# DaehwanKimLab/tophat

Measured on AMD Instinct MI355X. Metric: paired reads/sec through segment_juncs+long_spanning_reads; junctions.bed diff=0, higher is better.
Workload: dtype u64

## Files before the change

### tophat_amd/csrc/thj_ctx.h

```cpp
#pragma once
#include <hip/hip_runtime.h>
#include <cstdint>
#include <utility>
#include <vector>

#include "../../include/thj.h"
#include "thj_core.h"
#include "thj_internal.h"
#include "thj_jbknown_core.h"

using thj::u64;

#define HIPCHK(expr)                                                                          \
    do {                                                                                      \
        hipError_t e__ = (expr);                                                              \
        if (e__ != hipSuccess) {                                                              \
            thj_set_error("%s: %s (%s:%d)", #expr, hipGetErrorString(e__), __FILE__, __LINE__); \
            return THJ_EHIP;                                                                  \
        }                                                                                     \
    } while (0)

struct OwnedSpanBatch {
    thj_span_batch desc;
    void* ptrs[8];
    size_t reads_infl_bytes;
};

template <class T> struct DevBuf { T* p = nullptr; int64_t cap = 0; void release() { (void)hipFree(p); p = nullptr; cap = 0; } };
struct JbStore { DevBuf<u64> w64; DevBuf<uint32_t> w32; DevBuf<unsigned long long> cnt; int64_t cap = 0; void release() { w64.release(); w32.release(); cnt.release(); cap = 0; } };
struct JbOcc; struct JbiOcc; struct JbfOcc; struct JbfUOcc; struct JbfJOcc; struct JbbRec;
struct JbState {
    int64_t want = 0, records = 0;
    jbk::ReadFilter flt{};
    struct Junc { JbStore tab; DevBuf<u64> sorted; DevBuf<JbOcc> occ; int64_t occ_used = 0; DevBuf<u64> known; int64_t n_known = 0; std::vector<thj_juncstat> rows; } junc;
    struct Indel { bool on = false; JbStore tab; DevBuf<JbiOcc> occ; int64_t occ_used = 0; std::vector<thj_insstat> ins; std::vector<thj_juncstat> del; } indel;
    struct Fus { bool on = false; int32_t anchor = 20, mismatches = 2, multireads = 2; JbStore tab; DevBuf<uint32_t> grp; int64_t groups = 0;
                 DevBuf<JbfOcc> focc; DevBuf<JbfUOcc> uocc; DevBuf<JbfJOcc> jocc; std::vector<thj_fusstat> rows; } fus;
    struct Best { bool on = false; int32_t max_multihits = 20, suppress = 0, max_penalty = 6; DevBuf<JbbRec> rec; DevBuf<u64> skey; DevBuf<uint8_t> keep;
                  DevBuf<unsigned long long> cnt; int64_t counts[4] = {0, 0, 0, 0}; } best;
};

struct CovState {
    int64_t n_blocks = 0; int32_t n_contigs = 0;
    DevBuf<u64> bits; DevBuf<int32_t> extent;
    unsigned long long* d_found = nullptr;
    DevBuf<uint32_t> rec_len; DevBuf<u64> rec_seq; int64_t n_reads = 0;
    uint32_t* d_ext_off = nullptr; DevBuf<u64> ext_val; DevBuf<u64> filter; u64 filter_mask = 0;
    struct List {
        u64 *key = nullptr, *key2 = nullptr; uint32_t *skip = nullptr, *skip2 = nullptr; int64_t cap = 0;
        void release() { (void)hipFree(key); (void)hipFree(key2); (void)hipFree(skip); (void)hipFree(skip2); *this = List(); }
    } list;
    DevBuf<thj_mx_cand> mx_cand; int64_t n_mx_cand = 0;
    int32_t min_intron = 0, max_intron = 0; bool pending = false;
    void release() {
        bits.release(); extent.release(); rec_len.release(); rec_seq.release(); ext_val.release(); filter.release(); list.release(); mx_cand.release();
        (void)hipFree(d_found); (void)hipFree(d_ext_off); *this = CovState();
    }
};

struct thj_ctx {
    int device = 0;
    hipStream_t stream = nullptr;
    bool own_stream = false;
    hipStream_t aux_stream[2] = {};
    double aux_ratio[2] = {0, 0}; bool aux_independent[2] = {false, false};
    const u64* d_blocks = nullptr; bool own_blocks = false;
    uint32_t* d_contig_blk = nullptr; int32_t* d_contig_len = nullptr;
    std::vector<uint32_t> h_contig_blk; std::vector<int64_t> h_lens;
    int32_t n_contigs = 0; int64_t n_blocks = 0;
    int64_t junc_cap = 0, indel_cap = 0;
    u64 *d_junc = nullptr, *d_del = nullptr, *d_ins_key = nullptr, *d_ins_val = nullptr;
    unsigned int* d_ovf = nullptr;
    unsigned long long* d_cnt = nullptr;
    u64 *d_junc_sorted = nullptr, *d_del_sorted = nullptr, *d_ins_key_sorted = nullptr, *d_ins_val_sorted = nullptr;
    u64 *d_tmp_keys = nullptr, *d_tmp_vals = nullptr, *d_tmp_keys2 = nullptr;
    int64_t out_cap_junc = 0, out_cap_indel = 0;
    unsigned long long* d_out_n = nullptr;
    unsigned long long* h_pinned = nullptr;
    void* d_sort_tmp = nullptr; size_t sort_tmp_bytes = 0;
    int64_t n_junc = 0, n_del = 0, n_ins = 0;
    hipEvent_t probe_ev = nullptr; bool probe_pending = false;
    uint8_t* d_fus_ignore = nullptr; int64_t n_fus_ignore = 0;
    struct SjSet {
        uint32_t* d_rescue_list = nullptr; int64_t rescue_list_cap = 0;
        uint32_t* d_many = nullptr;
        void* d_lists = nullptr; size_t lists_cap = 0;
        int32_t* d_rescue_slots = nullptr;
        hipEvent_t ev_flat = nullptr, ev_side = nullptr;
    } sj_set[2];
    uint32_t* d_junc_bucket = nullptr; int64_t n_junc_buckets = 0;
    u64* d_span_cat = nullptr;
    u64* d_span_junc = nullptr; int64_t n_span_junc = 0; int64_t cap_span_junc = 0;
    u64* d_span_ins_key = nullptr; uint32_t* d_span_ins_seq = nullptr; int64_t n_span_ins = 0; int64_t cap_span_ins = 0;
    void* d_huge_ws = nullptr; uint32_t* d_huge_list = nullptr; int huge_blocks = 0, huge_list_cap = 0;
    void* d_span_fus = nullptr; int64_t n_span_fus = 0; int64_t cap_span_fus = 0;
    void* d_aln_pool = nullptr; void* d_aln_sorted = nullptr; int64_t aln_cap = 0;
    u64* d_aln_keys = nullptr;
    unsigned long long* d_aln_count = nullptr; unsigned int* d_span_status = nullptr;
    int64_t n_alns = 0, n_ovf = 0, span_reads = 0, ovf_cap = 0;
    uint8_t* d_nrec = nullptr;
    std::vector<thj_aln> h_alns;
    struct SpanSet { uint32_t* d_worklist = nullptr; int64_t worklist_cap = 0; void* d_ent = nullptr; int64_t ent_cap = 0; void* d_joined = nullptr; int64_t joined_cap = 0; uint32_t* d_defer = nullptr; int64_t defer_cap = 0; };
    SpanSet span_set[2]; int span_last_set = 0;
    bool span_t0_pending = false; int64_t span_t0_n[2] = {0, 0}; hipEvent_t span_t0_prof[2][32] = {};
    hipEvent_t span_ev[10] = {};
    bool span_profile = false;
    std::vector<std::pair<hipEvent_t, hipEvent_t>> span_prof_events;
    CovState cov;
    thj_fusion* d_fus = nullptr; unsigned long long* d_fus_count = nullptr; int64_t fus_cap = 0;
    hipEvent_t fus_probe_ev = nullptr; bool fus_probe_pending = false;
    std::vector<thj_fusion> h_fusions;
    thj_fusion* d_fus_out = nullptr; int64_t n_fus_out = 0;
    bool h_fus_stale = false;
    struct DevBlock { void* p; size_t cap; bool used; };
    std::vector<DevBlock> dev_cache; size_t dev_cache_bytes = 0;
    void* d_ing0 = nullptr; size_t ing_cap0 = 0; void* d_ing1 = nullptr; size_t ing_cap1 = 0;
    thj_juncdb_target* d_juncdb = nullptr; int64_t n_juncdb = 0;
    bool juncdb_has_fus = false, juncdb_fusion_on = false;
    uint8_t* d_bam = nullptr; size_t bam_cap = 0; int64_t bam_bytes = 0;
    void* d_bam_tmp = nullptr; size_t bam_tmp_cap = 0;
    uint8_t* d_contig_names = nullptr; uint32_t* d_contig_name_off = nullptr; uint32_t* d_contig_name_sorted = nullptr; int32_t n_contig_names = 0;
    void* d_infl_tmp = nullptr; size_t infl_tmp_cap = 0;
    JbState jb;
    struct thj_comm* xchg = nullptr;
    bool profile = false;
    bool serial_launch = false;
    std::vector<std::pair<hipEvent_t, hipEvent_t>> prof_events;
    std::vector<hipEvent_t> prof_all; std::vector<int> prof_sets;
    std::vector<hipEvent_t> event_pool;
};
template <class T, class C>
static inline int grow_device_buffer(T*& ptr, C& cap, C new_cap, size_t bytes) {
    if (ptr) HIPCHK(hipDeviceSynchronize());
    (void)hipFree(ptr); ptr = nullptr; cap = 0;
    HIPCHK(hipMalloc((void**)&ptr, bytes));
    cap = new_cap;
    return THJ_OK;
}
static inline int ensure_sort_tmp(struct thj_ctx* c, size_t need) {
    return need > c->sort_tmp_bytes ? grow_device_buffer(c->d_sort_tmp, c->sort_tmp_bytes, need, need) : THJ_OK;
}
template <class Run>
static inline int run_with_sort_tmp(struct thj_ctx* c, Run run) {
    size_t need = 0;
    HIPCHK(run(nullptr, need));
    if (const int e = ensure_sort_tmp(c, need)) return e;
    size_t bytes = c->sort_tmp_bytes;
    HIPCHK(run(c->d_sort_tmp, bytes));
    return THJ_OK;
}
template <class T>
static inline int read_device_value(struct thj_ctx* c, const T* d, T* h) {
    HIPCHK(hipMemcpyAsync(h, d, sizeof(T), hipMemcpyDeviceToHost, c->stream));
    HIPCHK(hipStreamSynchronize(c->stream));
    return THJ_OK;
}
struct DevTemps {
    std::vector<void**> slots;
    DevTemps() = default; DevTemps(const DevTemps&) = delete;
    template <class T> hipError_t alloc(T*& p, size_t bytes) { p = nullptr; slots.push_back((void**)&p); return hipMalloc((void**)&p, bytes); }
    ~DevTemps() { for (void** p : slots) { (void)hipFree(*p); *p = nullptr; } }
};
hipEvent_t thj_get_event(struct thj_ctx* c);
int thj_ensure_aux_streams(struct thj_ctx* c, int need);
void thj_warm_span(hipStream_t s); void thj_warm_ingest(hipStream_t s); void thj_warm_bamout(hipStream_t s);
int thj_dev_alloc(struct thj_ctx* c, void** out, size_t bytes);
void thj_dev_release(struct thj_ctx* c, void* p);
void thj_dev_cache_free(struct thj_ctx* c);
void thj_span_free(struct thj_ctx* c);
int thj_span_compact_device(struct thj_ctx* c, void** d_out);
void thj_bamout_free(struct thj_ctx* c);
struct thj_reported_recs { thj_aln* recs; int64_t n; const int64_t* ins_off; uint8_t* ins_bases; int64_t n_groups; uint32_t resume_member, resume_skip; };
// ... 5 lines not shown
```

### tophat_amd/csrc/thj_segjuncs.hip

```cpp
#include <hip/hip_runtime.h>
#include <hipcub/hipcub.hpp>

#include <cstdio>
#include <cstdlib>
#include <algorithm>
#include <cstring>
#include <cstddef>
#include <chrono>
#include <vector>

#include "../../include/thj.h"
#include "thj_core.h"
#include "thj_fusion_block.h"
#include "thj_internal.h"

using namespace thj;

static_assert(sizeof(thj_hit) == 16 && sizeof(Hit) == 16, "hit layout");
static_assert(sizeof(thj_params) == sizeof(Params), "params layout");




static constexpr u64 EMPTY = ~0ull;
// ... 1205 lines not shown
    if (!c->probe_pending || hipEventQuery(c->probe_ev) != hipSuccess) return THJ_OK;
    c->probe_pending = false;
    const unsigned long long* n = &c->h_pinned[32];
    const bool gj = n[CNT_JUNC] * 5 > (unsigned long long)c->junc_cap * 2;
    const bool gi = (n[CNT_DEL] > n[CNT_INS] ? n[CNT_DEL] : n[CNT_INS]) * 5 > (unsigned long long)c->indel_cap * 2;
    return (gj || gi) ? grow_tables(c, gj, gi) : THJ_OK;
}

extern "C" int thj_segjuncs_configure(thj_ctx* c, int64_t junc_capacity, int64_t indel_capacity) {
    if (!c || junc_capacity < 1 || indel_capacity < 1) { thj_set_error("thj_segjuncs_configure: bad argument"); return THJ_EINVAL; }
    HIPCHK(hipSetDevice(c->device));
    HIPCHK(hipStreamSynchronize(c->stream));
    int rc = alloc_tables(c, junc_capacity, indel_capacity);
    if (rc) return rc;
    return reset_tables_async(c);
}

extern "C" int thj_segjuncs_reset_async(thj_ctx* c) {
    if (!c) { thj_set_error("null ctx"); return THJ_EINVAL; }
    HIPCHK(hipSetDevice(c->device));
    return reset_tables_async(c);
}

static int check_params(const thj_params* p, const thj_seg_batch* b) {
    if (p->segment_length < 8 || p->segment_length > 64) {
        thj_set_error("segment_length %d unsupported by the device path (8..64: the 8 bases either side of a segment boundary "
                      "that make a support read must lie inside the segments, segment_juncs.cpp:3580-3584; a 2L read piece and an "
                      "L+16 support read must fit one 128-bit plane word)", p->segment_length);
        return THJ_EINVAL;
    }
    if (p->max_insertion_length > 6 || p->max_insertion_length < 0) { thj_set_error("max_insertion_length %d unsupported (0..6)", p->max_insertion_length); return THJ_EINVAL; }
    if (p->max_deletion_length < 0 || p->max_deletion_length > 1000000) { thj_set_error("max_deletion_length out of range"); return THJ_EINVAL; }
    if (p->max_segment_intron + p->segment_length + 64 >= (1 << 29)) { thj_set_error("max_segment_intron too large for the packed key"); return THJ_EINVAL; }
    if (b->nseg < 1 || b->nseg > 16) { thj_set_error("nseg %d unsupported (1..16)", b->nseg); return THJ_EINVAL; }
    if (b->words_per_plane < 1 || b->words_per_plane > 8) { thj_set_error("words_per_plane %d unsupported (1..8: reads of up to 512 bases)", b->words_per_plane); return THJ_EINVAL; }
    if (b->n_reads < 0 || (int64_t)b->n_reads + b->ordinal_base >= (1ll << 29)) { thj_set_error("batch too large: read ordinals must stay below 2^29"); return THJ_EINVAL; }
    return THJ_OK;
}

int thj_dev_alloc(thj_ctx* c, void** out, size_t bytes) {
    if (bytes < 256) bytes = 256;
    int best = -1;
    for (size_t i = 0; i < c->dev_cache.size(); ++i) {
        const thj_ctx::DevBlock& b = c->dev_cache[i];
        if (!b.used && b.cap >= bytes && b.cap <= 2 * bytes + 65536 && (best < 0 || b.cap < c->dev_cache[(size_t)best].cap)) best = (int)i;
    }
    if (best >= 0) { c->dev_cache[(size_t)best].used = true; *out = c->dev_cache[(size_t)best].p; return THJ_OK; }
    if (c->dev_cache_bytes > ((size_t)16 << 30)) {
        for (size_t i = 0; i < c->dev_cache.size();) {
            if (!c->dev_cache[i].used) { hipFree(c->dev_cache[i].p); c->dev_cache_bytes -= c->dev_cache[i].cap; c->dev_cache.erase(c->dev_cache.begin() + (ptrdiff_t)i); }
            else ++i;
        }
    }
    const size_t cap = bytes + bytes / 8;
    void* p = nullptr;
    HIPCHK(hipMalloc(&p, cap));
    c->dev_cache.push_back({p, cap, true});
    c->dev_cache_bytes += cap;
    *out = p;
    return THJ_OK;
}
void thj_dev_release(thj_ctx* c, void* p) {
    if (!p) return;
    for (auto& b : c->dev_cache) if (b.p == p) { b.used = false; return; }
    hipFree(p);
}
void thj_dev_cache_free(thj_ctx* c) {
    for (auto& b : c->dev_cache) hipFree(b.p);
    c->dev_cache.clear(); c->dev_cache_bytes = 0;
}

hipEvent_t thj_get_event(thj_ctx* c) {
    if (!c->event_pool.empty()) { hipEvent_t e = c->event_pool.back(); c->event_pool.pop_back(); return e; }
    hipEvent_t e;
    hipEventCreate(&e);
    return e;
}


struct SjGeom {
    int n_tiles, grid, seg_cap;
    int tmax; size_t xcap;
    int rgrid, mgrid; bool wide;
    int64_t slots() const { return (int64_t)grid * seg_cap; }
    int64_t rescue_slice_words() const { return slots(); }             int64_t rescue_shared_words() const { return 2 * (int64_t)MANY_CAP; }
    int64_t rescue_words() const { return rescue_slice_words() + rescue_shared_words() + MAX_LISTS; }
    size_t tq_bytes() const { return (size_t)slots() * tmax * 16; }    size_t xq_bytes() const { return xcap * 16; }
    size_t frl_bytes() const { return (size_t)slots() * 32; }
    size_t te_bytes() const { return (size_t)slots() * tmax * 4; }
    size_t gen_bytes() const { return (size_t)slots() * 4; }           size_t xe_bytes() const { return xcap * 4; }
    size_t cnt_bytes() const { return (size_t)grid * 12; }
    size_t lists_bytes() const { return tq_bytes() + xq_bytes() + frl_bytes() + te_bytes() + gen_bytes() + xe_bytes() + cnt_bytes() + 512; }
};
static SjGeom sj_geometry(const Params& p, const DevBatch& b) {
    SjGeom q{};
    q.n_tiles = (b.n_reads + TPB - 1) / TPB;
    q.grid = q.n_tiles < 256 * 8 - 1 ? q.n_tiles : 256 * 8 - 1;
    q.seg_cap = (q.n_tiles + q.grid - 1) / q.grid * TPB;
    q.tmax = (b.nseg > 2 ? b.nseg - 2 : 0) + (b.nseg - 1 > 2 * FLAT_MATES ? b.nseg - 1 : 2 * FLAT_MATES);
    q.xcap = (size_t)2 * (size_t)b.n_reads > ((size_t)1 << 20) ? (size_t)2 * (size_t)b.n_reads : ((size_t)1 << 20);
    if (getenv("THJ_XTASK_CAP")) q.xcap = (size_t)atoll(getenv("THJ_XTASK_CAP"));
    q.rgrid = q.grid < RESCUE_GRID ? q.grid : RESCUE_GRID; q.mgrid = q.n_tiles < MID_GRID ? q.n_tiles : MID_GRID; q.wide = p.segment_length > 32;
    return q;
}
static constexpr size_t SJ_MANY_BYTES = 32 + (size_t)MANY_CAP * 8;
static constexpr size_t SJ_SLOTS_BYTES = 16 + (size_t)HEAVY_CAP * 4;
static int ensure_sj_set(thj_ctx* c, int set, const SjGeom& q, bool mates) {
    thj_ctx::SjSet& ss = c->sj_set[set];
    const bool grow_rescue = ss.rescue_list_cap < q.rescue_words(), grow_lists = ss.lists_cap < q.lists_bytes();
    if ((grow_rescue || grow_lists) && getenv("THJ_TRACE"))
        fprintf(stderr, "[stage 1] scratch set %d grows:%s%s (%lld words, %zu bytes needed)\n", set, grow_rescue ? " rescue list" : "", grow_lists ? " list block" : "", (long long)q.rescue_words(), q.lists_bytes());
    if (grow_rescue) { const int rc = grow_device_buffer(ss.d_rescue_list, ss.rescue_list_cap, q.rescue_words(), (size_t)q.rescue_words() * 4); if (rc) return rc; }
    if (!ss.d_many) HIPCHK(hipMalloc((void**)&ss.d_many, SJ_MANY_BYTES));
    if (mates && !ss.d_rescue_slots) HIPCHK(hipMalloc((void**)&ss.d_rescue_slots, SJ_SLOTS_BYTES));
    if (grow_lists) { const size_t cap = q.lists_bytes() + q.lists_bytes() / 8; return grow_device_buffer(ss.d_lists, ss.lists_cap, cap, cap); }
    return THJ_OK;
}

struct SjPlan {
    int set; bool serial;
    hipStream_t s_main;
    hipStream_t s_side;
    hipEvent_t ev_flat;
    hipEvent_t ev_side;
    hipEvent_t m_flat[2];
};
static int sj_plan(thj_ctx* c, int set, SjPlan& pl) {
    static const bool serial_env = getenv("THJ_SJ_SERIAL") && atoi(getenv("THJ_SJ_SERIAL")) != 0;
    thj_ctx::SjSet& ss = c->sj_set[set];
    pl = SjPlan{}; pl.set = set; pl.serial = serial_env || c->serial_launch; pl.s_main = pl.s_side = c->stream;
    if (pl.serial) return THJ_OK;
    if (const int rc = thj_ensure_aux_streams(c, set + 1)) return rc;
    if (!ss.ev_flat) { HIPCHK(hipEventCreateWithFlags(&ss.ev_flat, hipEventDisableTiming)); HIPCHK(hipEventCreateWithFlags(&ss.ev_side, hipEventDisableTiming)); }
    pl.s_side = c->aux_stream[set]; pl.ev_flat = ss.ev_flat; pl.ev_side = ss.ev_side;
    return THJ_OK;
}

struct SjView { Genome g; Params p; DevBatch b; Tables t; RescueList rl; SjLists sl; XTasks x; SjGeom q; unsigned long long* cnt; };
static int sj_view(thj_ctx* c, const thj_params* tp, const thj_seg_batch* db, int set, SjView& v) {
    v.g = Genome{c->d_blocks, c->d_contig_blk, c->d_contig_len, c->n_contigs};
    memcpy(&v.p, tp, sizeof v.p); memcpy(&v.b, db, sizeof v.b);
    v.t = Tables{c->d_junc, (u64)c->junc_cap - 1, c->d_del, (u64)c->indel_cap - 1, c->d_ins_key, c->d_ins_val,
                 (u64)c->indel_cap - 1, junc_list(c), del_list(c), ins_list(c), c->d_ovf, c->d_cnt};
    v.cnt = c->d_cnt;
#ifdef THJ_EXP
    { int f = getenv("THJ_EXP_FLAGS") ? atoi(getenv("THJ_EXP_FLAGS")) : 0; HIPCHK(hipMemcpyToSymbol(HIP_SYMBOL(thj_exp_flags), &f, sizeof f)); }
#endif
    const SjGeom q = v.q = sj_geometry(v.p, v.b);
    if (const int rc = ensure_sj_set(c, set, q, v.b.mate_off != nullptr)) return rc;
    const thj_ctx::SjSet& ss = c->sj_set[set];
    unsigned int* const counts = (unsigned int*)ss.d_many;
    static const int many_min = getenv("THJ_MANY_HITS") ? atoi(getenv("THJ_MANY_HITS")) : MID_HITS;
    RescueList& rl = v.rl;
    rl.list = ss.d_rescue_list; rl.blk_cnt = ss.d_rescue_list + q.rescue_slice_words() + q.rescue_shared_words(); rl.seg_cap = q.seg_cap; rl.own_slice = q.grid;
    rl.many_min = many_min; rl.mid_min = many_min < GEN_HITS ? many_min : GEN_HITS;
    rl.many_count = counts; rl.many_list = ss.d_many + 8;
    rl.heavy_count = (unsigned int*)ss.d_rescue_slots; rl.heavy_list = ss.d_rescue_slots ? (uint32_t*)ss.d_rescue_slots + 4 : nullptr; rl.slot_pool = nullptr;
    SjLists& sl = v.sl; XTasks& x = v.x;
    char* at = (char*)ss.d_lists;
    auto take = [&at](size_t bytes) { char* const piece = at; at += bytes; return piece; };
    sl.tq = (uint4*)take(q.tq_bytes());            x.q = (uint4*)take(q.xq_bytes());
    sl.frl = (uint4*)take(q.frl_bytes());          sl.te = (uint32_t*)take(q.te_bytes());
    sl.gen = (uint32_t*)take(q.gen_bytes());       x.e = (uint32_t*)take(q.xe_bytes());
    sl.task_cnt = (unsigned int*)take(q.cnt_bytes()); sl.frl_cnt = sl.task_cnt + q.grid; sl.gen_cnt = sl.frl_cnt + q.grid;
    sl.task_cap = q.seg_cap * q.tmax;
    sl.mid_count = counts + 2; sl.mid_list = ss.d_many + 8 + MANY_CAP;
    x.count = counts + 3; x.cap = (unsigned int)(q.xcap < 0xFFFFFFFFull ? q.xcap : 0xFFFFFFFFull); x.ovf = c->d_ovf + 3;
    return THJ_OK;
}

static void launch_sj_flat(const SjView& v, hipStream_t s) {
    const dim3 grid((unsigned)v.q.grid), tpb(TPB);
    if (v.b.nseg <= 4) hipLaunchKernelGGL(thj_k_sj_flat<4>, grid, tpb, 0, s, v.p, v.b, v.rl, v.sl, v.cnt);
    else if (v.b.nseg <= 8) hipLaunchKernelGGL(thj_k_sj_flat<8>, grid, tpb, 0, s, v.p, v.b, v.rl, v.sl, v.cnt);
    else hipLaunchKernelGGL(thj_k_sj_flat<16>, grid, tpb, 0, s, v.p, v.b, v.rl, v.sl, v.cnt);
}
template <int HITS, int T, bool SLICED, int G>
static void launch_sj_general(const SjView& v, int grid, hipStream_t s) {
    if (v.b.nseg <= 8) hipLaunchKernelGGL((thj_k_sj_general<HITS, T, SLICED, 9, G>), dim3((unsigned)grid), dim3(T), 0, s, v.p, v.b, v.rl, v.sl, v.x, v.cnt);
    else hipLaunchKernelGGL((thj_k_sj_general<HITS, T, SLICED, 17, G>), dim3((unsigned)grid), dim3(T), 0, s, v.p, v.b, v.rl, v.sl, v.x, v.cnt);
}
static void launch_sj_tasks_list(const SjView& v, hipStream_t s) {
    if (v.q.wide) hipLaunchKernelGGL(thj_k_sj_tasks_list<true>, dim3(v.q.rgrid), dim3(TPB), 0, s, v.g, v.p, v.b, v.t, v.x);
    else hipLaunchKernelGGL(thj_k_sj_tasks_list<false>, dim3(v.q.rgrid), dim3(TPB), 0, s, v.g, v.p, v.b, v.t, v.x);
}
static void launch_sj_tasks(const SjView& v, hipStream_t s) {
    if (v.q.wide) hipLaunchKernelGGL(thj_k_sj_tasks<true>, dim3(v.q.grid), dim3(TPB), 0, s, v.g, v.p, v.b, v.t, v.sl);
    else hipLaunchKernelGGL(thj_k_sj_tasks<false>, dim3(v.q.grid), dim3(TPB), 0, s, v.g, v.p, v.b, v.t, v.sl);
}

static constexpr int SJ_PROF_N = 8;
static hipEvent_t sj_mark(thj_ctx* c, hipStream_t s) { if (!c->profile) return nullptr; hipEvent_t e = thj_get_event(c); hipEventRecord(e, s); c->prof_all.push_back(e); return e; }

static int sj_launch_flat(thj_ctx* c, SjPlan& pl, const SjView& v) {
    const thj_ctx::SjSet& ss = c->sj_set[pl.set];
    HIPCHK(hipMemsetAsync(ss.d_many, 0, 32, pl.s_main));
    HIPCHK(hipMemsetAsync(v.rl.blk_cnt + v.q.grid, 0, 4, pl.s_main));
    if (v.b.mate_off) HIPCHK(hipMemsetAsync(ss.d_rescue_slots, 0, 16, pl.s_main));
    pl.m_flat[0] = sj_mark(c, pl.s_main);
    launch_sj_flat(v, pl.s_main);
    pl.m_flat[1] = sj_mark(c, pl.s_main);
    if (!pl.serial) { HIPCHK(hipEventRecord(pl.ev_flat, pl.s_main)); HIPCHK(hipStreamWaitEvent(pl.s_side, pl.ev_flat, 0)); }
    HIPCHK(hipGetLastError());
    return THJ_OK;
}

static int sj_launch_rest(thj_ctx* c, const SjPlan& pl, const SjView& v) {
    const SjGeom& q = v.q;
    const hipStream_t sm = pl.s_main, sa = pl.s_side;
    hipEvent_t b0 = sj_mark(c, sa);
    hipLaunchKernelGGL(thj_k_segjuncs_shared, dim3(q.rgrid), dim3(TPB), 0, sa, v.p, v.b, v.rl, v.x, v.cnt);
    hipEvent_t b1 = sj_mark(c, sa);
    launch_sj_general<MID_HITS, MID_T, false, MID_G>(v, q.mgrid, sa);
    hipEvent_t c1 = sj_mark(c, sa);
    launch_sj_general<GEN_HITS, TPB, true, GEN_G>(v, q.grid, sa);
    hipEvent_t a1 = sj_mark(c, sa);
    if (v.b.mate_off) {
        hipLaunchKernelGGL(thj_k_segjuncs_rescue, dim3(q.rgrid), dim3(TPB), 0, sa, v.g, v.p, v.b, v.rl, q.grid + 1, v.x, v.cnt);
        hipLaunchKernelGGL(thj_k_segjuncs_rescue_shared, dim3(q.rgrid), dim3(TPB), 0, sa, v.g, v.p, v.b, v.rl, v.x, v.cnt);
    }
    hipEvent_t a4 = sj_mark(c, sa);
    launch_sj_tasks_list(v, sa);
    hipEvent_t a5 = sj_mark(c, sa);
    if (!pl.serial) HIPCHK(hipEventRecord(pl.ev_side, sa));
    hipEvent_t m2 = sj_mark(c, sm);
    if (v.b.mate_off) hipLaunchKernelGGL(thj_k_sj_rescue_flat, dim3(q.grid), dim3(TPB), 0, sm, v.g, v.p, v.b, v.sl, q.seg_cap, v.cnt, v.sl.mid_count + 2);
    hipEvent_t m3 = sj_mark(c, sm);
    launch_sj_tasks(v, sm);
    hipEvent_t m4 = sj_mark(c, sm);
    if (c->profile) {
        const std::pair<hipEvent_t, hipEvent_t> spans[SJ_PROF_N] = {{pl.m_flat[0], pl.m_flat[1]}, {c1, a1}, {b1, c1}, {b0, b1}, {a1, a4}, {a4, a5}, {m2, m3}, {m3, m4}};
        c->prof_events.insert(c->prof_events.end(), spans, spans + SJ_PROF_N);
        c->prof_sets.push_back(pl.set);
    }
    HIPCHK(hipGetLastError());
    return THJ_OK;
}

static int sj_join(const SjPlan& pl) { if (!pl.serial) HIPCHK(hipStreamWaitEvent(pl.s_main, pl.ev_side, 0)); return THJ_OK; }
static int sj_probe(thj_ctx* c) {
    if (!c->probe_ev) HIPCHK(hipEventCreateWithFlags(&c->probe_ev, hipEventDisableTiming));
    if (!c->probe_pending) {
        HIPCHK(hipMemcpyAsync(&c->h_pinned[32], c->d_cnt, CNT_N * sizeof(unsigned long long), hipMemcpyDeviceToHost, c->stream));
        HIPCHK(hipEventRecord(c->probe_ev, c->stream));
        c->probe_pending = true;
    }
    return THJ_OK;
}

extern "C" int thj_segjuncs_run_async(thj_ctx* c, const thj_params* tp, const thj_seg_batch* db) {
    if (!c || !tp || !db) { thj_set_error("thj_segjuncs_run_async: null argument"); return THJ_EINVAL; }
    if (!c->d_blocks) { thj_set_error("no genome resident: call thj_genome_upload/adopt first"); return THJ_ESTATE; }
    int rc = check_params(tp, db);
    if (rc) return rc;
    HIPCHK(hipSetDevice(c->device));
    if (db->n_reads == 0) return THJ_OK;
    if ((rc = maybe_grow_tables(c))) return rc;
    SjPlan pl; SjView v;
    if ((rc = sj_plan(c, 0, pl)) || (rc = sj_view(c, tp, db, 0, v)) || (rc = sj_launch_flat(c, pl, v)) || (rc = sj_launch_rest(c, pl, v)) || (rc = sj_join(pl))) return rc;
    return sj_probe(c);
}

extern "C" int thj_segjuncs_run_pair_async(thj_ctx* c, const thj_params* tp0, const thj_seg_batch* db0, const thj_params* tp1, const thj_seg_batch* db1) {
    if (!c || !tp0 || !db0 || !tp1 || !db1) { thj_set_error("thj_segjuncs_run_pair_async: null argument"); return THJ_EINVAL; }
    if (!c->d_blocks) { thj_set_error("no genome resident: call thj_genome_upload/adopt first"); return THJ_ESTATE; }
    int rc = check_params(tp0, db0);
    if (rc || (rc = check_params(tp1, db1))) return rc;
    HIPCHK(hipSetDevice(c->device));
    if ((rc = maybe_grow_tables(c))) return rc;
    const thj_params* const tp[2] = {tp0, tp1}; const thj_seg_batch* const db[2] = {db0, db1};
    SjPlan pl[2]; SjView v[2];
    for (int k = 0; k < 2; ++k) if (db[k]->n_reads && ((rc = sj_plan(c, k, pl[k])) || (rc = sj_view(c, tp[k], db[k], k, v[k])))) return rc;
    for (int k = 0; k < 2; ++k) if (db[k]->n_reads && (rc = sj_launch_flat(c, pl[k], v[k]))) return rc;
    if (db0->n_reads && (rc = sj_launch_rest(c, pl[0], v[0]))) return rc;
    if (db1->n_reads && (rc = sj_launch_rest(c, pl[1], v[1]))) { if (db0->n_reads) sj_join(pl[0]); return rc; }
    for (int k = 0; k < 2; ++k) if (db[k]->n_reads && (rc = sj_join(pl[k]))) return rc;
    return (db0->n_reads || db1->n_reads) ? sj_probe(c) : THJ_OK;
}

extern "C" int thj_profile_serial(thj_ctx* c, int on) {
    if (!c) { thj_set_error("null ctx"); return THJ_EINVAL; }
    HIPCHK(hipSetDevice(c->device));
    HIPCHK(hipStreamSynchronize(c->stream));
    c->serial_launch = on != 0;
    return THJ_OK;
}

extern "C" int thj_profile_segjuncs(thj_ctx* c, int enable, double* avg_ms, int64_t* launches, double* stats) {
    if (!c) { thj_set_error("null ctx"); return THJ_EINVAL; }
    HIPCHK(hipSetDevice(c->device));
    HIPCHK(hipStreamSynchronize(c->stream));
    double sum[SJ_PROF_N] = {0};
    const size_t n = c->prof_events.size() / SJ_PROF_N;
    for (size_t i = 0; i < c->prof_events.size(); ++i) {
// ... 465 lines not shown
```

### tophat_amd/csrc/thj_span.hip

```cpp
#include <hip/hip_runtime.h>
#include <hipcub/hipcub.hpp>

#include <cstdio>
#include <algorithm>
#include <cstdlib>
#include <cstring>
#include <cstddef>
#include <chrono>
#include <vector>

#include "../../include/thj.h"
#include "thj_span_core.h"
#include "thj_span_fusion.h"
#include "thj_ctx.h"
#include "thj_scan.h"

using namespace thj;


static_assert(sizeof(thj_span_hit) == 32 && sizeof(SpanHit) == 32, "span hit layout");
static_assert(sizeof(thj_aln) == 128 && sizeof(OutAln) == 128 && sizeof(thj_aln_slot) == 128 && offsetof(thj_aln_slot, cigar_hi) == 64, "aln layout");

struct DevSpanBatch {
    int32_t n_reads, nseg, W, qual_stride;
// ... 181 lines not shown
    for (int k = 0; k < IPT; ++k) { s_off[tid * IPT + k] = excl; excl += v[k]; }
    if (tid == 0) s_off[NS] = total;
    __syncthreads();
    return total;
}
__device__ __forceinline__ int slice_of(const unsigned int* s_off, int G, unsigned int i) {
    int lo = 0, hi = G;
    while (hi - lo > 1) { const int mid = (lo + hi) >> 1; if (s_off[mid] <= i) lo = mid; else hi = mid; }
    return lo;
}

template <int MS, int WPE = 4>
__global__ __launch_bounds__(256, WPE) void thj_k_stitch(Genome g, Params p, SpanSets S, DevSpanBatch b, RecSink sink, Tiers t, int G) {
    extern __shared__ uint4 lds_stage[];
    constexpr int NC = lean_classes(MS);
    __shared__ unsigned int s_off[NC * MAX_SLICES + 1];
    __shared__ unsigned int s_rec, s_fwd;
    if (threadIdx.x == 0) { s_rec = 0; s_fwd = 0; }
    unsigned int n_fwd = 0;
    SpanHitHead* stage = (SpanHitHead*)lds_stage + (size_t)threadIdx.x * b.nseg;
    const unsigned int total = slice_offsets<256, NC * MAX_SLICES>(t.blk_lean, NC * G, s_off);
    for (unsigned int i = blockIdx.x * 256 + threadIdx.x; i < total; i += gridDim.x * 256) {
        int sl = slice_of(s_off, NC * G, i);
        const int r = (int)t.wl_lean[(int64_t)sl * t.chunk + (i - s_off[sl])];
        int st = span_read_lean<MS>(g, p, S, b.hits, b.seg_off + (size_t)r * b.nseg, b.nseg, b.planes + (size_t)r * 3 * b.W, b.W,
                                (int)b.read_len[r], b.quals + (size_t)r * b.qual_stride, (uint32_t)r, stage, sink);
        if (st == SPAN_INCOMPAT) st = p.fusion_search ? SPAN_NEED_GENERIC : SPAN_OK;
        const bool fwd = st == SPAN_NEED_GENERIC;
        if (!fwd) { sink.done((uint32_t)r); if (st) atomicAdd(&sink.status[st], 1u); }
        sl %= G;
        for (unsigned long long todo = __ballot(fwd); todo;) {
            const int leader = __ffsll((long long)todo) - 1;
            const int sl_l = __shfl(sl, leader);
            const unsigned long long same = __ballot(fwd && sl == sl_l);
            const int lane = (int)(threadIdx.x & 63u);
            unsigned int base = 0;
            if (lane == leader) base = atomicAdd(&t.blk_multi[sl_l], (unsigned int)__popcll(same));
            base = (unsigned int)__shfl((int)base, leader);
            if (fwd && sl == sl_l) {
                t.wl_multi[(int64_t)sl * t.chunk + base + (unsigned int)__popcll(same & (lane ? (~0ull >> (64 - lane)) : 0ull))] = (uint32_t)r;
                ++n_fwd;
            }
            todo &= ~same;
        }
    }
    if (sink.acc) atomicAdd(&s_rec, (unsigned int)sink.acc);
    if (n_fwd) atomicAdd(&s_fwd, n_fwd);
    __syncthreads();
    if (threadIdx.x == 0 && s_rec) atomicAdd(sink.total, (unsigned long long)s_rec);
    if (threadIdx.x == 0 && s_fwd) atomicAdd(&t.counters[1], s_fwd);
}

struct LdsChainHits {
    const Q16* col;
    __device__ __forceinline__ SpanHit operator[](int s) const {
        const Q16 a = col[(2 * s) * 256], b = col[(2 * s + 1) * 256];
        SpanHit h;
        h.ref_id = a.x; h.left = (int32_t)a.y; h.meta = a.z; h.cigar[0] = a.w;
        h.cigar[1] = b.x; h.cigar[2] = b.y; h.cigar[3] = b.z; h.cigar[4] = b.w;
        return h;
    }
};
struct LdsChainHits6 {
    const Q16* col; const uint2* col2;
    __device__ __forceinline__ SpanHit operator[](int s) const {
        const Q16 a = col[s * 256]; const uint2 b = col2[s * 256];
        SpanHit h;
        h.ref_id = a.x; h.left = (int32_t)a.y; h.meta = a.z; h.cigar[0] = a.w;
        h.cigar[1] = b.x; h.cigar[2] = b.y; h.cigar[3] = 0; h.cigar[4] = 0;
        return h;
    }
};
struct ChainLists {
    const ChainEntry* ent; const unsigned int* blk_cnt; int G, chunk;
    const ChainEntry* ent2; const unsigned int* n2; int G2; unsigned int cap2, slice2;
    Q16* ja; Q16* jb; Q16* jc;
};
__device__ __forceinline__ unsigned int chain_block_counts(const ChainLists& L, int blk, unsigned int (&c)[SPAN_LEAN_CLASSES]) {
    unsigned int total = 0;
#pragma unroll
    for (int k = 0; k < SPAN_LEAN_CLASSES; ++k) { c[k] = L.blk_cnt[k * L.G + blk]; total += c[k]; }
    return total;
}
__device__ __forceinline__ unsigned int chain_dense_count(const ChainLists& L) { const unsigned int n = *L.n2; return n < L.cap2 ? n : L.cap2; }
struct DeferList {
    uint32_t* idx; unsigned int* cnt; uint4* tiles; unsigned int tslice;
    __device__ __forceinline__ uint4* tiles_of(const ChainLists& L, unsigned int w) const {
        const unsigned int ta = (unsigned int)L.chunk / 64u;
        return tiles + ((int)w < L.G ? (u64)w * ta : (u64)L.G * ta + (u64)(w - (unsigned int)L.G) * tslice);
    }
};
template <bool ABUT>
__device__ __forceinline__ int join_compute(const Genome& g, const Params& p, const SpanSets& S, const SpanHit* hits, const u64* planes, int W,
                                            Q16* s_rec, const ChainEntry* entry, uint32_t& r, uint32_t& meta, RAln& res, RegRead* rw = nullptr) {
    Q16 rec[2 * CHAIN_MAXSEG];
    if (ABUT) { if (!chain_entry_fetch(hits, planes, W, entry, r, meta, rec, rw)) return LJ_NONE; }
    else {
        const Q16* src = (const Q16*)entry;
        const Q16 e0 = src[0], e1 = src[1];
        r = e0.x; meta = e0.y;
        if (r == JOINED_PAD) return LJ_NONE;
        const uint32_t hi[CHAIN_MAXSEG] = {e1.x, e1.y, e1.z, e1.w};
#pragma unroll
        for (int k = 0; k < CHAIN_MAXSEG; ++k) { const Q16* hp = (const Q16*)(hits + hi[k]); rec[2 * k] = hp[0]; rec[2 * k + 1] = hp[1]; }
    }
    if (ABUT) {
        bool wide = false;
#pragma unroll
        for (int k = 0; k < CHAIN_MAXSEG; ++k) wide = wide || (rec[2 * k].z >> 24) > 3u;
        if (wide) return LJ_DEFER;
        uint2* s2 = (uint2*)(s_rec + CHAIN_MAXSEG * 256);
#pragma unroll
        for (int k = 0; k < CHAIN_MAXSEG; ++k) { s_rec[k * 256 + threadIdx.x] = rec[2 * k]; s2[k * 256 + threadIdx.x] = make_uint2(rec[2 * k + 1].x, rec[2 * k + 1].y); }
        const LdsChainHits6 ch{s_rec + threadIdx.x, s2 + threadIdx.x};
        return chain_join<ABUT>(g, p, S, ch, meta, planes + (u64)r * (uint32_t)(3 * W), W, res);
    }
#pragma unroll
    for (int k = 0; k < 2 * CHAIN_MAXSEG; ++k) s_rec[k * 256 + threadIdx.x] = rec[k];
    const LdsChainHits ch{s_rec + threadIdx.x};
    return chain_join<ABUT>(g, p, S, ch, meta, planes + (u64)r * (uint32_t)(3 * W), W, res);
}
__device__ __forceinline__ void join_punt(const Tiers& t, uint32_t r, uint32_t meta) {
    if (chain_k(meta) > 1) atomicExch(&t.status[5], 1u);
    else {
        const uint32_t gb = r / (uint32_t)t.chunk;
        t.wl_gen[(u64)gb * (uint32_t)t.chunk + atomicAdd(&t.blk_gen[gb], 1u)] = r;
        atomicAdd(&t.counters[2], 1u);
    }
}
__device__ __forceinline__ void join_store(const ChainLists& L, u64 at, uint32_t r, uint32_t meta, int jr, const RAln& res) {
    if (r == JOINED_PAD) { L.ja[at] = Q16{JOINED_PAD, 0u, 0u, 0u}; return; }
    Q16 ja, jb, jc;
    joined_pack(res, r, chain_nsegs(meta) == 1, chain_q(meta), chain_k(meta), ja, jb, jc);
    if (jr != LJ_OK) ja.w = joined_none_meta(chain_q(meta), chain_k(meta));
    L.ja[at] = ja;
    if (jr == LJ_OK) { L.jb[at] = jb; if (res.n > 4) L.jc[at] = jc; }
}
__device__ __forceinline__ bool join_prepare_direct(const Genome& g, const Params& p, const DevSpanBatch& b, uint32_t r, uint32_t meta, const RegRead& rw, RAln& res, Extras& e) {
    Q16 ja, jb, jc;
    joined_pack(res, r, chain_nsegs(meta) == 1, chain_q(meta), chain_k(meta), ja, jb, jc);
    return joined_prepare(g, p, ja, jb, jc, b.planes, b.W, rw, chain_rl(meta), b.quals, b.qual_stride, res, e);
}
__device__ __forceinline__ const ChainEntry* chain_locate(const unsigned int (&c)[SPAN_LEAN_CLASSES], const ChainLists& L, int blk, unsigned int i) {
    unsigned int cls = 0, local = i;
#pragma unroll
    for (int k = 0; k < SPAN_LEAN_CLASSES - 1; ++k) { const bool next = cls == (unsigned int)k && local >= c[k]; local -= next ? c[k] : 0u; cls += next ? 1u : 0u; }
    return L.ent + (u64)(cls * (unsigned int)L.G + (unsigned int)blk) * (unsigned int)L.chunk + local;
}

struct FinishSink {
    uint4* dst;
    __device__ __forceinline__ void emit_words(const uint32_t* w) {
        const bool tail = slot_needs_tail(w);
#pragma unroll
        for (int k = 0; k < 4; ++k) dst[k] = make_uint4(slot_word(w, 4 * k, tail), slot_word(w, 4 * k + 1, tail), slot_word(w, 4 * k + 2, tail), slot_word(w, 4 * k + 3, tail));
        if (tail) {
#pragma unroll
            for (int k = 4; k < 8; ++k) dst[k] = make_uint4(slot_word(w, 4 * k, true), slot_word(w, 4 * k + 1, true), slot_word(w, 4 * k + 2, true), slot_word(w, 4 * k + 3, true));
        }
    }
};
__device__ __forceinline__ unsigned int finish_emit(const RecSink& sink, bool real, uint32_t r, int q, int kp, bool emit, const RAln& res, const Extras& e) {
    const int lane = (int)(threadIdx.x & 63u);
    const unsigned long long m = __ballot(emit);
    const unsigned long long below = lane ? (~0ull >> (64 - lane)) : 0ull;
    const unsigned long long gmask = (~0ull >> (64 - kp)) << (lane - q);
// ... 56 lines not shown
        const u64 base = (u64)blk * (uint32_t)L.chunk;
        for (unsigned int i0 = 0; i0 < total; i0 += 256) {
            const unsigned int i = i0 + threadIdx.x;
            const int jr = join_finish_one(g, p, S, b, sink, L, t, s_rec, i < total ? chain_locate(c, L, blk, i) : nullptr, base + i, acc, gdef);
            if (jr == LJ_DEFER) D.idx[base + atomicAdd(&s_qn, 1u)] = i;
            const unsigned long long tm = __ballot(gdef);
            if (tm && lane == 0) tiles[atomicAdd(&s_tn, 1u)] = make_uint4(i, (uint32_t)tm, (uint32_t)(tm >> 32), 0u);
        }
    } else {
        const unsigned int j = blockIdx.x - (unsigned int)L.G, n2 = chain_dense_count(L);
        const u64 jbase = (u64)L.G * (uint32_t)L.chunk;
        for (unsigned int i0 = j * 256u; i0 < n2; i0 += (unsigned int)L.G2 * 256u) {
            const unsigned int i = i0 + threadIdx.x;
            const int jr = join_finish_one(g, p, S, b, sink, L, t, s_rec, i < n2 ? L.ent2 + i : nullptr, jbase + i, acc, gdef);
            if (jr == LJ_DEFER) D.idx[jbase + (u64)j * L.slice2 + atomicAdd(&s_qn, 1u)] = i;
            const unsigned long long tm = __ballot(gdef);
            if (tm && lane == 0) tiles[atomicAdd(&s_tn, 1u)] = make_uint4(i, (uint32_t)tm, (uint32_t)(tm >> 32), 0u);
        }
    }
    if (acc) atomicAdd(&s_nrec, acc);
    __syncthreads();
    if (threadIdx.x == 0) {
        D.cnt[blockIdx.x] = s_qn;
        D.cnt[L.G + L.G2 + blockIdx.x] = s_tn;
        if (s_nrec) atomicAdd(sink.total, (unsigned long long)s_nrec);
    }
}
__device__ __forceinline__ void join_entry(const Genome& g, const Params& p, const SpanSets& S, const DevSpanBatch& b, const ChainLists& L, const Tiers& t,
                                           Q16* s_rec, const ChainEntry* entry, u64 at) {
    uint32_t r, meta;
    RAln res;
    const int jr = join_compute<false>(g, p, S, b.hits, b.planes, b.W, s_rec, entry, r, meta, res);
    join_store(L, at, r, meta, jr, res);
    if (jr == LJ_PUNT) join_punt(t, r, meta);
}
template <int WPE>
__global__ __launch_bounds__(256, WPE) void thj_k_join_closure(Genome g, Params p, SpanSets S, DevSpanBatch b, ChainLists L, Tiers t, DeferList D) {
    __shared__ Q16 s_rec[2 * CHAIN_MAXSEG * 256];
    const unsigned int n = D.cnt[blockIdx.x];
    if ((int)blockIdx.x < L.G) {
        const int blk = (int)blockIdx.x;
        unsigned int c[SPAN_LEAN_CLASSES];
        chain_block_counts(L, blk, c);
        for (unsigned int k = threadIdx.x; k < n; k += 256) {
            const unsigned int i = D.idx[(u64)blk * (uint32_t)L.chunk + k];
            join_entry(g, p, S, b, L, t, s_rec, chain_locate(c, L, blk, i), (u64)blk * (uint32_t)L.chunk + i);
        }
    } else {
        const unsigned int j = blockIdx.x - (unsigned int)L.G;
        const u64 jbase = (u64)L.G * (uint32_t)L.chunk;
        for (unsigned int k = threadIdx.x; k < n; k += 256) {
            const unsigned int i = D.idx[jbase + (u64)j * L.slice2 + k];
            join_entry(g, p, S, b, L, t, s_rec, L.ent2 + i, jbase + i);
        }
    }
}

__device__ __forceinline__ unsigned int finish_one(const Genome& g, const Params& p, const DevSpanBatch& b, const RecSink& sink, const ChainLists& L, bool has, u64 at) {
    Q16 ja{JOINED_PAD, 0u, 0u, 0u};
    if (has) ja = L.ja[at];
    const bool real = ja.x != JOINED_PAD;
    RAln res; Extras e;
    bool emit = false;
    if (real && joined_n(ja.w) > 0) {
        const Q16 jb = L.jb[at];
        const int rl = (int)b.read_len[ja.x];
        const u64* rp = b.planes + (u64)ja.x * (uint32_t)(3 * b.W);
        RegRead rw;
#pragma unroll
        for (int i = 0; i < 6; ++i) rw.v[i] = 0;
        if (b.W == 2) {
#pragma unroll
            for (int i = 0; i < 6; ++i) rw.v[i] = rp[i];
        } else if (b.W == 1) { rw.v[0] = rp[0]; rw.v[2] = rp[1]; rw.v[4] = rp[2]; }
        Q16 jc{0u, 0u, 0u, 0u};
        if (joined_n(ja.w) > 4) jc = L.jc[at];
        emit = joined_prepare<0>(g, p, ja, jb, jc, b.planes, b.W, rw, rl, b.quals, b.qual_stride, res, e);
    }
    return finish_emit(sink, real, ja.x, joined_q(ja.w), chains_padded(joined_k(ja.w)), emit, res, e);
}
template <int WPE>
__global__ __launch_bounds__(256, WPE) void thj_k_finish(Genome g, Params p, DevSpanBatch b, RecSink sink, ChainLists L, DeferList D) {
    __shared__ unsigned int s_rec;
    if (threadIdx.x == 0) s_rec = 0;
    __syncthreads();
    const unsigned int n = D.cnt[L.G + L.G2 + blockIdx.x];
    const uint4* const tiles = D.tiles_of(L, blockIdx.x);
    const u64 ebase = (u64)((int)blockIdx.x < L.G ? blockIdx.x : (unsigned int)L.G) * (uint32_t)L.chunk;
    const unsigned int lane = threadIdx.x & 63u;
    unsigned int acc = 0;
    for (unsigned int k = threadIdx.x >> 6; k < n; k += 4) {
        const uint4 tl = tiles[k];
        const unsigned long long m = ((unsigned long long)tl.z << 32) | tl.y;
        acc += finish_one(g, p, b, sink, L, ((m >> lane) & 1ull) != 0ull, ebase + tl.x + lane);
    }
    if (acc) atomicAdd(&s_rec, acc);
    __syncthreads();
    if (threadIdx.x == 0 && s_rec) atomicAdd(sink.total, (unsigned long long)s_rec);
}

static constexpr int CH_TPB = 128;
struct LdsHitTab {
    const Q16* col;
    __device__ __forceinline__ SpanHitHead head(int j) const { const Q16 v = col[j * CH_TPB]; return SpanHitHead{v.x, (int32_t)v.y, v.z, v.w}; }
};
__global__ __launch_bounds__(CH_TPB) void thj_k_chains(Params p, DevSpanBatch b, Tiers t, ChainEntry* ent2, unsigned int* n2, unsigned int cap2, uint32_t* wl_pack, unsigned int* blk_pack, int G) {
    __shared__ Q16 s_head[CHAINS_MAXHITS * CH_TPB];
    __shared__ unsigned int s_base;
    typedef hipcub::BlockScan<u64, CH_TPB> Scan;
    __shared__ typename Scan::TempStorage tmp;
    const int tid = (int)threadIdx.x;
    for (int blk = blockIdx.x; blk < G; blk += gridDim.x) {
        const unsigned int n_b = t.blk_multi[blk];
        unsigned int pack_n = 0;
        for (unsigned int j0 = 0; j0 < n_b; j0 += CH_TPB) {
            const unsigned int j = j0 + (unsigned int)tid;
            const bool has = j < n_b;
            const uint32_t r = has ? t.wl_multi[(u64)blk * (uint32_t)t.chunk + j] : 0u;
            int k = 0, nsegs = 0;
            uint32_t sel[CHAINS_MAX]; int q[CHAINS_MAX];
#pragma unroll
            for (int c = 0; c < CHAINS_MAX; ++c) { sel[c] = 0; q[c] = 0; }
            uint32_t sof0 = 0;
            if (has) {
                const uint32_t* so = b.seg_off + (u64)r * (uint32_t)b.nseg;
                uint32_t sof[CHAIN_MAXSEG + 1];
#pragma unroll
                for (int s = 0; s <= CHAIN_MAXSEG; ++s) sof[s] = s <= b.nseg ? so[s <= b.nseg ? s : 0] : 0u;
                {
                    bool open = true;
#pragma unroll
                    for (int s = 0; s < CHAIN_MAXSEG; ++s) { open = open && s < b.nseg && sof[s + 1] > sof[s]; nsegs += open ? 1 : 0; }
                }
                sof0 = sof[0];
                uint32_t last_so = sof[0], end_so = sof[0];
#pragma unroll
                for (int s = 1; s <= CHAIN_MAXSEG; ++s) { last_so = (s == nsegs - 1) ? sof[s] : last_so; end_so = (s == nsegs) ? sof[s] : end_so; }
                bool ok = nsegs > 0 && (load_head(b.hits, b.heads, (u64)last_so).z & SH_END) != 0;
                if (ok && p.bowtie2) {
#pragma unroll
                    for (int s = 0; s < CHAIN_MAXSEG; ++s) ok = ok && !(s < nsegs && (int)(sof[s + 1] - sof[s]) > p.max_seg_multihits);
                }
                if (ok) {
                    const uint32_t nh = end_so - sof[0];
                    k = CHAINS_DECLINE;
                    if (nh <= (uint32_t)CHAINS_MAXHITS) {
                        for (uint32_t h0 = 0; h0 < nh; h0 += 8) {
                            Q16 hq[8];
#pragma unroll
                            for (int x = 0; x < 8; ++x) hq[x] = load_head(b.hits, b.heads, (u64)sof[0] + (h0 + x < nh ? h0 + x : nh - 1));
#pragma unroll
                            for (int x = 0; x < 8; ++x)
                                if (h0 + x < nh) s_head[(h0 + x) * CH_TPB + tid] = Q16{hq[x].x, hq[x].y, hq[x].z, (uint32_t)pack_hit_right(hq[x], b.hits, (u64)sof[0] + h0 + x)};
                        }
                        uint32_t off[CHAIN_MAXSEG + 1];
#pragma unroll
                        for (int s = 0; s <= CHAIN_MAXSEG; ++s) off[s] = sof[s] - sof[0];
                        const LdsHitTab tab{s_head + tid};
                        k = chains_discover(p, tab, off, nsegs, sel, q);
                    }
                }
            }
            const int kp = k > 0 ? chains_padded(k) : 0;
            const bool declined = has && k == CHAINS_DECLINE;
            const u64 mine = (kp == 8 ? 1ull : 0ull) | (kp == 4 ? 1ull << 8 : 0ull) | (kp == 2 ? 1ull << 16 : 0ull) | (kp == 1 ? 1ull << 24 : 0ull) | (declined ? 1ull << 32 : 0ull);
            u64 excl, tot;
            Scan(tmp).ExclusiveSum(mine, excl, tot);
            const unsigned int N8 = (unsigned int)(tot & 255u), N4 = (unsigned int)((tot >> 8) & 255u), N2 = (unsigned int)((tot >> 16) & 255u), N1 = (unsigned int)((tot >> 24) & 255u);
            const unsigned int ND = (unsigned int)((tot >> 32) & 255u);
            const unsigned int T = 8u * N8 + 4u * N4 + 2u * N2 + N1, T8 = (T + 7u) & ~7u;
            if (tid == 0) s_base = T8 ? atomicAdd(n2, T8) : 0u;
// ... 1096 lines not shown
```

Baseline: 2.144 billion.

## Size stage-1 grids from occupancy queries and reorder finish-kernel slice mapping

Queries resident workgroups per CU for each stage-1 kernel once and caches the result in the context. The segjuncs grid cap now comes from MAX_LISTS-1 (overridable by THJ_SJ_GRID) instead of a fixed constant. The shared kernel's grid is clamped to the resident capacity rather than the rescue grid. The finish kernel maps block indices so the dense-chain slices run first, which puts the likely heavier blocks at the start of the launch. The aim is to fit grid sizes to what the device can hold at once and to reduce tail imbalance, at the cost of different slice counts and scratch sizes.

Measured after the change: 2.148 billion, median of 2. Within noise of the previous version (+0.2%).

```diff
diff --git a/tophat_amd/csrc/thj_ctx.h b/tophat_amd/csrc/thj_ctx.h
--- a/tophat_amd/csrc/thj_ctx.h
+++ b/tophat_amd/csrc/thj_ctx.h
@@ -88,6 +88,11 @@
         int32_t* d_rescue_slots = nullptr;
         hipEvent_t ev_flat = nullptr, ev_side = nullptr;
     } sj_set[2];
+    struct SjResident {
+        bool known = false;
+        int flat[3] = {}, tasks[2] = {}, gen[2] = {}, mid[2] = {}, tasks_list[2] = {};
+        int rescue_flat = 0, shared = 0, rescue = 0, rescue_shared = 0;
+    } sj_res;
     uint32_t* d_junc_bucket = nullptr; int64_t n_junc_buckets = 0;
     u64* d_span_cat = nullptr;
     u64* d_span_junc = nullptr; int64_t n_span_junc = 0; int64_t cap_span_junc = 0;
diff --git a/tophat_amd/csrc/thj_segjuncs.hip b/tophat_amd/csrc/thj_segjuncs.hip
--- a/tophat_amd/csrc/thj_segjuncs.hip
+++ b/tophat_amd/csrc/thj_segjuncs.hip
@@ -1311,6 +1311,7 @@
     int n_tiles, grid, seg_cap;
     int tmax; size_t xcap;
     int rgrid, mgrid; bool wide;
+    int g_shared;
     int64_t slots() const { return (int64_t)grid * seg_cap; }
     int64_t rescue_slice_words() const { return slots(); }             int64_t rescue_shared_words() const { return 2 * (int64_t)MANY_CAP; }
     int64_t rescue_words() const { return rescue_slice_words() + rescue_shared_words() + MAX_LISTS; }
@@ -1321,15 +1322,49 @@
     size_t cnt_bytes() const { return (size_t)grid * 12; }
     size_t lists_bytes() const { return tq_bytes() + xq_bytes() + frl_bytes() + te_bytes() + gen_bytes() + xe_bytes() + cnt_bytes() + 512; }
 };
-static SjGeom sj_geometry(const Params& p, const DevBatch& b) {
+template <class K> static int sj_resident_of(K kernel, int threads, int cus, int& out) {
+    int per_cu = 0;
+    HIPCHK(hipOccupancyMaxActiveBlocksPerMultiprocessor(&per_cu, (const void*)kernel, threads, 0));
+    if (per_cu < 1) { thj_set_error("stage 1: the runtime reports a kernel that no CU can hold"); return THJ_ESTATE; }
+    out = per_cu * cus;
+    return THJ_OK;
+}
+static int sj_resident(thj_ctx* c) {
+    thj_ctx::SjResident& R = c->sj_res;
+    if (R.known) return THJ_OK;
+    int cus = 0, rc = 0;
+    HIPCHK(hipDeviceGetAttribute(&cus, hipDeviceAttributeMultiprocessorCount, c->device));
+    if (cus < 1) { thj_set_error("stage 1: the device reports no CU"); return THJ_ESTATE; }
+    if ((rc = sj_resident_of(thj_k_sj_flat<4>, TPB, cus, R.flat[0])) || (rc = sj_resident_of(thj_k_sj_flat<8>, TPB, cus, R.flat[1])) ||
+        (rc = sj_resident_of(thj_k_sj_flat<16>, TPB, cus, R.flat[2])) ||
+        (rc = sj_resident_of(thj_k_sj_tasks<false>, TPB, cus, R.tasks[0])) || (rc = sj_resident_of(thj_k_sj_tasks<true>, TPB, cus, R.tasks[1])) ||
+        (rc = sj_resident_of(thj_k_sj_general<GEN_HITS, TPB, true, 9, GEN_G>, TPB, cus, R.gen[0])) ||
+        (rc = sj_resident_of(thj_k_sj_general<GEN_HITS, TPB, true, 17, GEN_G>, TPB, cus, R.gen[1])) ||
+        (rc = sj_resident_of(thj_k_sj_general<MID_HITS, MID_T, false, 9, MID_G>, MID_T, cus, R.mid[0])) ||
+        (rc = sj_resident_of(thj_k_sj_general<MID_HITS, MID_T, false, 17, MID_G>, MID_T, cus, R.mid[1])) ||
+        (rc = sj_resident_of(thj_k_sj_tasks_list<false>, TPB, cus, R.tasks_list[0])) || (rc = sj_resident_of(thj_k_sj_tasks_list<true>, TPB, cus, R.tasks_list[1])) ||
+        (rc = sj_resident_of(thj_k_sj_rescue_flat, TPB, cus, R.rescue_flat)) || (rc = sj_resident_of(thj_k_segjuncs_shared, TPB, cus, R.shared)) ||
+        (rc = sj_resident_of(thj_k_segjuncs_rescue, TPB, cus, R.rescue)) || (rc = sj_resident_of(thj_k_segjuncs_rescue_shared, TPB, cus, R.rescue_shared))) return rc;
+    if (getenv("THJ_TRACE"))
+        fprintf(stderr, "[stage 1] resident workgroups on %d CUs: flat %d/%d/%d, tasks %d/%d, general %d/%d, second instance %d/%d, tasks_list %d/%d, rescue_flat %d, shared %d, rescue %d, rescue_shared %d\n",
+                cus, R.flat[0], R.flat[1], R.flat[2], R.tasks[0], R.tasks[1], R.gen[0], R.gen[1], R.mid[0], R.mid[1], R.tasks_list[0], R.tasks_list[1], R.rescue_flat, R.shared, R.rescue, R.rescue_shared);
+    R.known = true;
+    return THJ_OK;
+}
+static int sj_forced_grid() { const char* e = getenv("THJ_SJ_GRID"); return e ? atoi(e) : 0; }
+static SjGeom sj_geometry(const thj_ctx::SjResident& R, const Params& p, const DevBatch& b) {
     SjGeom q{};
     q.n_tiles = (b.n_reads + TPB - 1) / TPB;
-    q.grid = q.n_tiles < 256 * 8 - 1 ? q.n_tiles : 256 * 8 - 1;
+    q.wide = p.segment_length > 32;
+    int slices = MAX_LISTS - 1;
+    if (const int forced = sj_forced_grid(); forced >= 1 && forced < slices) slices = forced;
+    q.grid = q.n_tiles < slices ? q.n_tiles : slices;
     q.seg_cap = (q.n_tiles + q.grid - 1) / q.grid * TPB;
     q.tmax = (b.nseg > 2 ? b.nseg - 2 : 0) + (b.nseg - 1 > 2 * FLAT_MATES ? b.nseg - 1 : 2 * FLAT_MATES);
     q.xcap = (size_t)2 * (size_t)b.n_reads > ((size_t)1 << 20) ? (size_t)2 * (size_t)b.n_reads : ((size_t)1 << 20);
     if (getenv("THJ_XTASK_CAP")) q.xcap = (size_t)atoll(getenv("THJ_XTASK_CAP"));
-    q.rgrid = q.grid < RESCUE_GRID ? q.grid : RESCUE_GRID; q.mgrid = q.n_tiles < MID_GRID ? q.n_tiles : MID_GRID; q.wide = p.segment_length > 32;
+    q.rgrid = q.grid < RESCUE_GRID ? q.grid : RESCUE_GRID; q.mgrid = q.n_tiles < MID_GRID ? q.n_tiles : MID_GRID;
+    q.g_shared = q.grid < R.shared ? q.grid : R.shared;
     return q;
 }
 static constexpr size_t SJ_MANY_BYTES = 32 + (size_t)MANY_CAP * 8;
@@ -1375,7 +1410,8 @@
 #ifdef THJ_EXP
     { int f = getenv("THJ_EXP_FLAGS") ? atoi(getenv("THJ_EXP_FLAGS")) : 0; HIPCHK(hipMemcpyToSymbol(HIP_SYMBOL(thj_exp_flags), &f, sizeof f)); }
 #endif
-    const SjGeom q = v.q = sj_geometry(v.p, v.b);
+    if (const int rc = sj_resident(c)) return rc;
+    const SjGeom q = v.q = sj_geometry(c->sj_res, v.p, v.b);
     if (const int rc = ensure_sj_set(c, set, q, v.b.mate_off != nullptr)) return rc;
     const thj_ctx::SjSet& ss = c->sj_set[set];
     unsigned int* const counts = (unsigned int*)ss.d_many;
@@ -1438,7 +1474,7 @@
     const SjGeom& q = v.q;
     const hipStream_t sm = pl.s_main, sa = pl.s_side;
     hipEvent_t b0 = sj_mark(c, sa);
-    hipLaunchKernelGGL(thj_k_segjuncs_shared, dim3(q.rgrid), dim3(TPB), 0, sa, v.p, v.b, v.rl, v.x, v.cnt);
+    hipLaunchKernelGGL(thj_k_segjuncs_shared, dim3(q.g_shared), dim3(TPB), 0, sa, v.p, v.b, v.rl, v.x, v.cnt);
     hipEvent_t b1 = sj_mark(c, sa);
     launch_sj_general<MID_HITS, MID_T, false, MID_G>(v, q.mgrid, sa);
     hipEvent_t c1 = sj_mark(c, sa);
diff --git a/tophat_amd/csrc/thj_span.hip b/tophat_amd/csrc/thj_span.hip
--- a/tophat_amd/csrc/thj_span.hip
+++ b/tophat_amd/csrc/thj_span.hip
@@ -287,6 +287,9 @@
     for (int k = 0; k < SPAN_LEAN_CLASSES; ++k) { c[k] = L.blk_cnt[k * L.G + blk]; total += c[k]; }
     return total;
 }
+__device__ __forceinline__ unsigned int chain_slice_of(const ChainLists& L) {
+    return blockIdx.x < (unsigned int)L.G2 ? (unsigned int)L.G + blockIdx.x : blockIdx.x - (unsigned int)L.G2;
+}
 __device__ __forceinline__ unsigned int chain_dense_count(const ChainLists& L) { const unsigned int n = *L.n2; return n < L.cap2 ? n : L.cap2; }
 struct DeferList {
     uint32_t* idx; unsigned int* cnt; uint4* tiles; unsigned int tslice;
@@ -509,11 +512,12 @@
 template <int WPE>
 __global__ __launch_bounds__(256, WPE) void thj_k_finish(Genome g, Params p, DevSpanBatch b, RecSink sink, ChainLists L, DeferList D) {
     __shared__ unsigned int s_rec;
+    const unsigned int w = chain_slice_of(L);
     if (threadIdx.x == 0) s_rec = 0;
     __syncthreads();
-    const unsigned int n = D.cnt[L.G + L.G2 + blockIdx.x];
-    const uint4* const tiles = D.tiles_of(L, blockIdx.x);
-    const u64 ebase = (u64)((int)blockIdx.x < L.G ? blockIdx.x : (unsigned int)L.G) * (uint32_t)L.chunk;
+    const unsigned int n = D.cnt[L.G + L.G2 + w];
+    const uint4* const tiles = D.tiles_of(L, w);
+    const u64 ebase = (u64)((int)w < L.G ? w : (unsigned int)L.G) * (uint32_t)L.chunk;
     const unsigned int lane = threadIdx.x & 63u;
     unsigned int acc = 0;
     for (unsigned int k = threadIdx.x >> 6; k < n; k += 4) {
```
